# Vidvox/hap

Measured on AMD Instinct MI355X. Metric: RGBA GB/s + frames/sec, 8K Hap Q encode+decode, higher is better.
Workload: dtype u8; 1 GPU; C4: 7680x4320 0x1, 24 chunks, Snappy, 60-frame stream, device-resident; fragment_index=True, parallelism=single GPU

## Files before the change

hap_amd/csrc/bc_encode_core.hpp:

```cpp
#pragma once
#include <hip/hip_runtime.h>
#include <stdint.h>

namespace hapbc {

constexpr int kFmtDXT1 = 0, kFmtDXT5 = 1, kFmtYCoCg = 2, kFmtRGTC1 = 3;
constexpr int kFmtYCoCgAlpha = 4;

__device__ __forceinline__ int mad24(int a, int b, int c)
{
    int r;
    asm("v_mad_i32_i24 %0, %1, %2, %3" : "=v"(r) : "v"(a), "v"(b), "v"(c));
    return r;
}
template <int K>
__device__ __forceinline__ int mad24k(int a, int c)
{
    int r;
    asm("v_mad_i32_i24 %0, %1, %2, %3" : "=v"(r) : "v"(a), "i"(K), "v"(c));
    return r;
}

__device__ __forceinline__ int quant5(int v) { int t = mad24k<31>(v, 128); return (t + (t >> 8)) >> 8; }
__device__ __forceinline__ int quant6(int v) { int t = mad24k<63>(v, 128); return (t + (t >> 8)) >> 8; }
__device__ __forceinline__ int expand5(int q) { return (q << 3) | (q >> 2); }
__device__ __forceinline__ int expand6(int q) { return (q << 2) | (q >> 4); }


__device__ __forceinline__ unsigned ramp_codes(unsigned w)
{
    return w ^ (~((w >> 1) | (w >> 2)) & 0x249249u);
}

__device__ __forceinline__ uint2 alpha_block(const int (&a)[16])
{
    int lo = a[0], hi = a[0];
#pragma unroll
    for (int i = 1; i < 16; i++) {
        lo = min(lo, a[i]);
        hi = max(hi, a[i]);
    }
    const int a0 = hi, a1 = lo;
    unsigned lo24 = 0, hi24 = 0;
    if (a0 != a1) {
        const int d = a0 - a1;
        unsigned q = (unsigned)(524288.0f * __builtin_amdgcn_rcpf((float)d));
        const int rem = 524288 - (int)__umul24(q, (unsigned)d);
        q += (rem >= d ? 1u : 0u) - (rem < 0 ? 1u : 0u);
        const unsigned m = q + 1u;
        const int neg_m14 = -(int)(14u * m);
        const int start = mad24(a0, (int)(14u * m), (int)__umul24((unsigned)max(d - 6, 0), m)) + (1 << 20);
#pragma unroll
        for (int i = 0; i < 16; i++) {
            const unsigned r1 = (unsigned)mad24(a[i], neg_m14, start) >> 20;
            if (i < 8)
                lo24 = __builtin_amdgcn_alignbit(r1, lo24, 3);
            else
                hi24 = __builtin_amdgcn_alignbit(r1, hi24, 3);
        }
        lo24 = ramp_codes(lo24 >> 8);
        hi24 = ramp_codes(hi24 >> 8);
    }
    const unsigned long long bits = (unsigned long long)lo24 | ((unsigned long long)hi24 << 24);
    const unsigned long long v = (unsigned long long)(unsigned)a0 | ((unsigned long long)(unsigned)a1 << 8) | (bits << 16);
    return make_uint2((unsigned)v, (unsigned)(v >> 32));
}

struct projection {
    unsigned adir;
    unsigned flip;
    int start;
    int top;
    unsigned m24;
};

__device__ __forceinline__ unsigned index_scale(unsigned len2)
{
    unsigned m = (unsigned)(50331648.0f * __builtin_amdgcn_rcpf((float)len2));
    const int rem = (int)(50331648u - m * len2);
    m += (rem >= (int)len2 ? 1u : 0u) - (rem < 0 ? 1u : 0u);
    return m;
}

template <int CHANNELS = 3>
__device__ __forceinline__ projection make_projection(unsigned p0, unsigned p1)
{
    projection pr;
    int dir[CHANNELS];
    unsigned adir = 0, flip = 0;
    int neg = 0, base = 0;
#pragma unroll
    for (int c = 0; c < CHANNELS; c++) {
        const int a = (int)((p0 >> (8 * c)) & 255u), b = (int)((p1 >> (8 * c)) & 255u);
        dir[c] = a - b;
        const int ad = abs(dir[c]);
        adir |= (unsigned)ad << (8 * c);
        flip |= (dir[c] < 0 ? 0xFFu : 0u) << (8 * c);
        neg += dir[c] < 0 ? ad : 0;
        base = mad24(b, dir[c], base);
    }
    const unsigned len2 = __builtin_amdgcn_udot4(adir, adir, 0u, false);
    const unsigned sixth = __umulhi(len2, 0xAAAAAAABu) >> 2;
    pr.adir = adir;
    pr.flip = flip;
    pr.start = (int)sixth - base - 255 * neg;
    pr.top = (int)(len2 + sixth);
    pr.m24 = index_scale(len2);
    return pr;
}

template <bool FLIPPED = false>
__device__ __forceinline__ unsigned project4(const unsigned (&px)[16], const projection &pr)
{
    unsigned pos2 = 0;
#pragma unroll
    for (int i = 0; i < 16; i++) {
        const unsigned q = FLIPPED ? px[i] : px[i] ^ pr.flip;
        const int t = (int)__builtin_amdgcn_udot4(q, pr.adir, (unsigned)pr.start, false);
        const int pos = min(max(__mul24(t, (int)pr.m24) >> 24, 0), 3);
        pos2 = __builtin_amdgcn_alignbit((unsigned)pos, pos2, 2);
    }
    const unsigned hi = pos2 & 0xAAAAAAAAu;
    const unsigned idx = (hi ^ ((pos2 << 1) & 0xAAAAAAAAu)) | ((~hi >> 1) & 0x55555555u);
    return idx;
}

__device__ __forceinline__ unsigned pack3(int a, int b, int c) { return (unsigned)a | ((unsigned)b << 8) | ((unsigned)c << 16); }

__device__ __forceinline__ unsigned expand_565(unsigned c, bool blue)
{
    return pack3(expand5(c >> 11), expand6((c >> 5) & 63), blue ? expand5(c & 31) : 0);
}

__device__ __forceinline__ uint2 colour_block(const unsigned (&px)[16])
{
    int lo[3] = {255, 255, 255}, hi[3] = {0, 0, 0};
#pragma unroll
    for (int i = 0; i < 16; i++) {
#pragma unroll
        for (int c = 0; c < 3; c++) {
            const int v = (int)((px[i] >> (8 * c)) & 255u);
            lo[c] = min(lo[c], v);
            hi[c] = max(hi[c], v);
        }
    }
    int cov_rg = 0, cov_bg = 0;
    const int mr = lo[0] + hi[0], mg = lo[1] + hi[1], mb = lo[2] + hi[2];
#pragma unroll
    for (int i = 0; i < 16; i++) {
        const int dr = 2 * (int)(px[i] & 255u) - mr;
        const int dg = 2 * (int)((px[i] >> 8) & 255u) - mg;
        const int db = 2 * (int)((px[i] >> 16) & 255u) - mb;
        cov_rg = mad24(dr, dg, cov_rg);
        cov_bg = mad24(db, dg, cov_bg);
    }
#pragma unroll
    for (int c = 0; c < 3; c++) {
        const int inset = (hi[c] - lo[c]) >> 4;
        lo[c] += inset;
        hi[c] -= inset;
    }
    const int ar = cov_rg < 0 ? lo[0] : hi[0], br = cov_rg < 0 ? hi[0] : lo[0];
    const int ab = cov_bg < 0 ? lo[2] : hi[2], bb = cov_bg < 0 ? hi[2] : lo[2];
    const unsigned qa = (unsigned)(quant5(ar) << 11 | quant6(hi[1]) << 5 | quant5(ab));
    const unsigned qb = (unsigned)(quant5(br) << 11 | quant6(lo[1]) << 5 | quant5(bb));
    const unsigned c0 = max(qa, qb), c1 = min(qa, qb);
    unsigned idx = 0;
    if (c0 != c1)
        idx = project4(px, make_projection(expand_565(c0, true), expand_565(c1, true)));
    return make_uint2(c0 | (c1 << 16), idx);
}

typedef unsigned short pk_u16 __attribute__((ext_vector_type(2)));
typedef short pk_i16 __attribute__((ext_vector_type(2)));

__device__ __forceinline__ uint2 ycocg_colour_block(const unsigned (&cc)[16])
{
    pk_u16 lo = __builtin_bit_cast(pk_u16, cc[0]), hi = lo;
#pragma unroll
    for (int i = 1; i < 16; i++) {
        const pk_u16 v = __builtin_bit_cast(pk_u16, cc[i]);
        lo = __builtin_elementwise_min(lo, v);
        hi = __builtin_elementwise_max(hi, v);
    }
    int lo_o = lo.x, hi_o = hi.x, lo_g = lo.y, hi_g = hi.y;
    const int m = max(max(128 - lo_o, hi_o - 128), max(128 - lo_g, hi_g - 128));
    const int s = m <= 31 ? 4 : (m <= 63 ? 2 : 1);
    int prod = 0;
    pk_u16 sums = {0, 0};
#pragma unroll
    for (int i = 0; i < 16; i++) {
        int r;
        asm("v_mad_i32_i16 %0, %1, %1, %2 op_sel:[0,1,0,0]" : "=v"(r) : "v"(cc[i]), "v"(prod));
        prod = r;
        sums += __builtin_bit_cast(pk_u16, cc[i]);
    }
    const int mo = lo_o + hi_o, mg = lo_g + hi_g;
    const int cov = 4 * prod - 2 * mg * (int)sums.x - 2 * mo * (int)sums.y + 16 * mo * mg;
    lo_o = (lo_o - 128) * s + 128; hi_o = (hi_o - 128) * s + 128;
    lo_g = (lo_g - 128) * s + 128; hi_g = (hi_g - 128) * s + 128;
    int ins = (hi_o - lo_o) >> 4; lo_o += ins; hi_o -= ins;
    ins = (hi_g - lo_g) >> 4; lo_g += ins; hi_g -= ins;
    const int ag = cov < 0 ? lo_g : hi_g, bg = cov < 0 ? hi_g : lo_g;
    const int qo_a = quant5(hi_o), qo_b = quant5(lo_o), qg_a = quant6(ag), qg_b = quant6(bg);
    const unsigned qa = (unsigned)(qo_a << 11 | qg_a << 5 | (s - 1));
    const unsigned qb = (unsigned)(qo_b << 11 | qg_b << 5 | (s - 1));
    const unsigned c0 = max(qa, qb), c1 = min(qa, qb);
    unsigned idx = 0;
    if (c0 != c1) {
        const bool sw = qa < qb;
        const int eo_a = expand5(qo_a), eo_b = expand5(qo_b), eg_a = expand6(qg_a), eg_b = expand6(qg_b);
        const int d_o = sw ? eo_b - eo_a : eo_a - eo_b, d_g = sw ? eg_b - eg_a : eg_a - eg_b;
        const int p1_o = sw ? eo_a : eo_b, p1_g = sw ? eg_a : eg_b;
        const unsigned len2 = (unsigned)mad24(d_o, d_o, __mul24(d_g, d_g));
        const int sixth = (int)(__umulhi(len2, 0xAAAAAAABu) >> 2);
        const unsigned m24 = index_scale(len2);
        const int centre = 128 - 128 * s;
        const int K = mad24(d_o, centre - p1_o, mad24(d_g, centre - p1_g, sixth));
        const pk_i16 dir2 = {(short)d_o, (short)d_g};
        constexpr int kDotOffset = 1 << 17;
        const unsigned sm = (unsigned)s * m24;
        const unsigned Km = (unsigned)(K - s * kDotOffset) * m24;
        unsigned pos2 = 0;
#pragma unroll
        for (int i = 0; i < 16; i++) {
            unsigned dot;
            asm("v_dot2_i32_i16 %0, %1, %2, %3\n\ts_nop 2" : "=v"(dot) : "v"(cc[i]), "v"(__builtin_bit_cast(unsigned, dir2)), "s"(kDotOffset));
            const int pos = min(max((int)(__umul24(dot, sm) + Km) >> 24, 0), 3);
            pos2 = __builtin_amdgcn_alignbit((unsigned)pos, pos2, 2);
        }
        const unsigned hi = pos2 & 0xAAAAAAAAu;
        idx = (hi ^ ((pos2 << 1) & 0xAAAAAAAAu)) | ((~hi >> 1) & 0x55555555u);
    }
    return make_uint2(c0 | (c1 << 16), idx);
}

template <int FMT>
__device__ __forceinline__ uint4 block_of(const unsigned (&p)[16])
{
    if (FMT == kFmtRGTC1) {
        int a[16];
#pragma unroll
        for (int i = 0; i < 16; i++)
            a[i] = (int)(p[i] >> 24);
        const uint2 ab = alpha_block(a);
        return make_uint4(ab.x, ab.y, 0u, 0u);
    } else if (FMT == kFmtDXT1) {
        unsigned px[16];
#pragma unroll
        for (int i = 0; i < 16; i++)
            px[i] = p[i] & 0x00FFFFFFu;
        const uint2 cb = colour_block(px);
        return make_uint4(cb.x, cb.y, 0u, 0u);
    } else if (FMT == kFmtDXT5) {
        int a[16];
        unsigned px[16];
#pragma unroll
        for (int i = 0; i < 16; i++) {
            a[i] = (int)(p[i] >> 24);
            px[i] = p[i] & 0x00FFFFFFu;
        }
        const uint2 ab = alpha_block(a), cb = colour_block(px);
        return make_uint4(ab.x, ab.y, cb.x, cb.y);
    } else {
        int y[16];
        unsigned cc[16];
#pragma unroll
        for (int i = 0; i < 16; i++) {
            const unsigned q = p[i];
            y[i] = (int)(__builtin_amdgcn_udot4(q, 0x00010201u, 2u, false) >> 2);
            const unsigned co2 = __builtin_amdgcn_udot4(q ^ 0x00FF0000u, 0x00010001u, 2u, false);
            const unsigned cg4 = __builtin_amdgcn_udot4(q ^ 0x00FF00FFu, 0x00010201u, 4u, false);
            const pk_u16 raw = __builtin_bit_cast(pk_u16, co2 | (cg4 << 16)), sh = {1, 2};
            cc[i] = __builtin_bit_cast(unsigned, (pk_u16)(raw >> sh));
        }
        const uint2 ab = alpha_block(y), cb = ycocg_colour_block(cc);
        return make_uint4(ab.x, ab.y, cb.x, cb.y);
    }
}

}
```

Measured before the change: 2557 GB/s.

## Recenter YCoCg chroma to signed values and batch clamped dot-product index projection

```diff
diff --git a/hap_amd/csrc/bc_encode_core.hpp b/hap_amd/csrc/bc_encode_core.hpp
--- a/hap_amd/csrc/bc_encode_core.hpp
+++ b/hap_amd/csrc/bc_encode_core.hpp
@@ -32,6 +32,7 @@
     return w ^ (~((w >> 1) | (w >> 2)) & 0x249249u);
 }
 
+template <int BIAS = 0>
 __device__ __forceinline__ uint2 alpha_block(const int (&a)[16])
 {
     int lo = a[0], hi = a[0];
@@ -62,7 +63,7 @@
         hi24 = ramp_codes(hi24 >> 8);
     }
     const unsigned long long bits = (unsigned long long)lo24 | ((unsigned long long)hi24 << 24);
-    const unsigned long long v = (unsigned long long)(unsigned)a0 | ((unsigned long long)(unsigned)a1 << 8) | (bits << 16);
+    const unsigned long long v = (unsigned long long)(unsigned)(a0 + (a1 << 8) + BIAS * 257) | (bits << 16);
     return make_uint2((unsigned)v, (unsigned)(v >> 32));
 }
 
@@ -109,20 +110,45 @@
     return pr;
 }
 
+#define HAPBC_CLAMPED_DOTS(OP)                                                                                           \
+    asm(OP " %0, %4, %8, %9\n\t" OP " %1, %5, %8, %9\n\t" OP " %2, %6, %8, %9\n\t" OP " %3, %7, %8, %9\n\t"              \
+        "v_med3_i32 %0, %0, 0, %10\n\tv_med3_i32 %1, %1, 0, %10\n\tv_med3_i32 %2, %2, 0, %10\n\tv_med3_i32 %3, %3, 0, %10" \
+        : "=&v"(t[0]), "=&v"(t[1]), "=&v"(t[2]), "=&v"(t[3])                                                             \
+        : "v"(q0), "v"(q1), "v"(q2), "v"(q3), "v"(dir), "v"(start), "v"(top))
+__device__ __forceinline__ void clamped_dot4(unsigned (&t)[4], unsigned q0, unsigned q1, unsigned q2, unsigned q3, unsigned dir, int start, int top)
+{
+    HAPBC_CLAMPED_DOTS("v_dot4_u32_u8");
+}
+__device__ __forceinline__ void clamped_dot2(unsigned (&t)[4], unsigned q0, unsigned q1, unsigned q2, unsigned q3, unsigned dir, int start, int top)
+{
+    HAPBC_CLAMPED_DOTS("v_dot2_i32_i16");
+}
+#undef HAPBC_CLAMPED_DOTS
+
+template <typename DOTS>
+__device__ __forceinline__ unsigned gather_indices(unsigned m24, DOTS dots)
+{
+    const unsigned m30 = m24 << 6;
+    unsigned pos2 = 0;
+#pragma unroll
+    for (int g = 3; g >= 0; g--) {
+        unsigned t[4];
+        dots(t, 4 * g);
+#pragma unroll
+        for (int k = 3; k >= 0; k--)
+            pos2 = __builtin_amdgcn_alignbit(pos2, t[k] * m30, 30);
+    }
+    const unsigned hi = pos2 & 0xAAAAAAAAu;
+    return (hi ^ ((pos2 << 1) & 0xAAAAAAAAu)) | ((~hi >> 1) & 0x55555555u);
+}
+
 template <bool FLIPPED = false>
 __device__ __forceinline__ unsigned project4(const unsigned (&px)[16], const projection &pr)
 {
-    unsigned pos2 = 0;
-#pragma unroll
-    for (int i = 0; i < 16; i++) {
-        const unsigned q = FLIPPED ? px[i] : px[i] ^ pr.flip;
-        const int t = (int)__builtin_amdgcn_udot4(q, pr.adir, (unsigned)pr.start, false);
-        const int pos = min(max(__mul24(t, (int)pr.m24) >> 24, 0), 3);
-        pos2 = __builtin_amdgcn_alignbit((unsigned)pos, pos2, 2);
-    }
-    const unsigned hi = pos2 & 0xAAAAAAAAu;
-    const unsigned idx = (hi ^ ((pos2 << 1) & 0xAAAAAAAAu)) | ((~hi >> 1) & 0x55555555u);
-    return idx;
+    return gather_indices(pr.m24, [&](unsigned (&t)[4], int i) {
+        clamped_dot4(t, FLIPPED ? px[i] : px[i] ^ pr.flip, FLIPPED ? px[i + 1] : px[i + 1] ^ pr.flip,
+                     FLIPPED ? px[i + 2] : px[i + 2] ^ pr.flip, FLIPPED ? px[i + 3] : px[i + 3] ^ pr.flip, pr.adir, pr.start, pr.top);
+    });
 }
 
 __device__ __forceinline__ unsigned pack3(int a, int b, int c) { return (unsigned)a | ((unsigned)b << 8) | ((unsigned)c << 16); }
@@ -176,29 +202,29 @@
 
 __device__ __forceinline__ uint2 ycocg_colour_block(const unsigned (&cc)[16])
 {
-    pk_u16 lo = __builtin_bit_cast(pk_u16, cc[0]), hi = lo;
+    pk_i16 lo = __builtin_bit_cast(pk_i16, cc[0]), hi = lo;
 #pragma unroll
     for (int i = 1; i < 16; i++) {
-        const pk_u16 v = __builtin_bit_cast(pk_u16, cc[i]);
+        const pk_i16 v = __builtin_bit_cast(pk_i16, cc[i]);
         lo = __builtin_elementwise_min(lo, v);
         hi = __builtin_elementwise_max(hi, v);
     }
     int lo_o = lo.x, hi_o = hi.x, lo_g = lo.y, hi_g = hi.y;
-    const int m = max(max(128 - lo_o, hi_o - 128), max(128 - lo_g, hi_g - 128));
+    const int m = max(max(-lo_o, hi_o), max(-lo_g, hi_g));
     const int s = m <= 31 ? 4 : (m <= 63 ? 2 : 1);
     int prod = 0;
-    pk_u16 sums = {0, 0};
+    pk_i16 sums = {0, 0};
 #pragma unroll
     for (int i = 0; i < 16; i++) {
         int r;
         asm("v_mad_i32_i16 %0, %1, %1, %2 op_sel:[0,1,0,0]" : "=v"(r) : "v"(cc[i]), "v"(prod));
         prod = r;
-        sums += __builtin_bit_cast(pk_u16, cc[i]);
+        sums += __builtin_bit_cast(pk_i16, cc[i]);
     }
     const int mo = lo_o + hi_o, mg = lo_g + hi_g;
     const int cov = 4 * prod - 2 * mg * (int)sums.x - 2 * mo * (int)sums.y + 16 * mo * mg;
-    lo_o = (lo_o - 128) * s + 128; hi_o = (hi_o - 128) * s + 128;
-    lo_g = (lo_g - 128) * s + 128; hi_g = (hi_g - 128) * s + 128;
+    lo_o = lo_o * s + 128; hi_o = hi_o * s + 128;
+    lo_g = lo_g * s + 128; hi_g = hi_g * s + 128;
     int ins = (hi_o - lo_o) >> 4; lo_o += ins; hi_o -= ins;
     ins = (hi_g - lo_g) >> 4; lo_g += ins; hi_g -= ins;
     const int ag = cov < 0 ? lo_g : hi_g, bg = cov < 0 ? hi_g : lo_g;
@@ -215,24 +241,24 @@
         const unsigned len2 = (unsigned)mad24(d_o, d_o, __mul24(d_g, d_g));
         const int sixth = (int)(__umulhi(len2, 0xAAAAAAABu) >> 2);
         const unsigned m24 = index_scale(len2);
-        const int centre = 128 - 128 * s;
-        const int K = mad24(d_o, centre - p1_o, mad24(d_g, centre - p1_g, sixth));
-        const pk_i16 dir2 = {(short)d_o, (short)d_g};
-        constexpr int kDotOffset = 1 << 17;
-        const unsigned sm = (unsigned)s * m24;
-        const unsigned Km = (unsigned)(K - s * kDotOffset) * m24;
-        unsigned pos2 = 0;
-#pragma unroll
-        for (int i = 0; i < 16; i++) {
-            unsigned dot;
-            asm("v_dot2_i32_i16 %0, %1, %2, %3\n\ts_nop 2" : "=v"(dot) : "v"(cc[i]), "v"(__builtin_bit_cast(unsigned, dir2)), "s"(kDotOffset));
-            const int pos = min(max((int)(__umul24(dot, sm) + Km) >> 24, 0), 3);
-            pos2 = __builtin_amdgcn_alignbit((unsigned)pos, pos2, 2);
-        }
-        const unsigned hi = pos2 & 0xAAAAAAAAu;
-        idx = (hi ^ ((pos2 << 1) & 0xAAAAAAAAu)) | ((~hi >> 1) & 0x55555555u);
+        const int K = mad24(d_o, 128 - p1_o, mad24(d_g, 128 - p1_g, sixth));
+        const unsigned dir2 = ((unsigned)(d_o * s) & 0xFFFFu) | ((unsigned)(d_g * s) << 16);
+        const int top = (int)len2 + sixth;
+        idx = gather_indices(m24, [&](unsigned (&t)[4], int i) { clamped_dot2(t, cc[i], cc[i + 1], cc[i + 2], cc[i + 3], dir2, K, top); });
     }
     return make_uint2(c0 | (c1 << 16), idx);
+}
+
+__device__ __forceinline__ void chroma4(unsigned (&raw)[4], int q0, int q1, int q2, int q3)
+{
+    unsigned co[4];
+    asm("v_dot4_i32_i8 %4, %8, %12, 1\n\tv_dot4_i32_i8 %0, %8, %13, 2\n\t"
+        "v_dot4_i32_i8 %5, %9, %12, 1\n\tv_dot4_i32_i8 %1, %9, %13, 2\n\t"
+        "v_dot4_i32_i8 %6, %10, %12, 1\n\tv_dot4_i32_i8 %2, %10, %13, 2\n\t"
+        "v_dot4_i32_i8 %7, %11, %12, 1\n\tv_dot4_i32_i8 %3, %11, %13, 2\n\t"
+        "v_perm_b32 %0, %0, %4, %14\n\tv_perm_b32 %1, %1, %5, %14\n\tv_perm_b32 %2, %2, %6, %14\n\tv_perm_b32 %3, %3, %7, %14"
+        : "=&v"(raw[0]), "=&v"(raw[1]), "=&v"(raw[2]), "=&v"(raw[3]), "=&v"(co[0]), "=&v"(co[1]), "=&v"(co[2]), "=&v"(co[3])
+        : "v"(q0), "v"(q1), "v"(q2), "v"(q3), "s"(0x00FF0001), "s"(0x00FF02FF), "s"(0x05040100));
 }
 
 template <int FMT>
@@ -267,14 +293,19 @@
         unsigned cc[16];
 #pragma unroll
         for (int i = 0; i < 16; i++) {
-            const unsigned q = p[i];
-            y[i] = (int)(__builtin_amdgcn_udot4(q, 0x00010201u, 2u, false) >> 2);
-            const unsigned co2 = __builtin_amdgcn_udot4(q ^ 0x00FF0000u, 0x00010001u, 2u, false);
-            const unsigned cg4 = __builtin_amdgcn_udot4(q ^ 0x00FF00FFu, 0x00010201u, 4u, false);
-            const pk_u16 raw = __builtin_bit_cast(pk_u16, co2 | (cg4 << 16)), sh = {1, 2};
-            cc[i] = __builtin_bit_cast(unsigned, (pk_u16)(raw >> sh));
-        }
-        const uint2 ab = alpha_block(y), cb = ycocg_colour_block(cc);
+            y[i] = (int)__builtin_amdgcn_udot4(p[i], 0x00010201u, (unsigned)(2 - 512), false) >> 2;
+        }
+#pragma unroll
+        for (int i = 0; i < 16; i += 4) {
+            unsigned raw[4];
+            chroma4(raw, (int)(p[i] ^ 0x80808080u), (int)(p[i + 1] ^ 0x80808080u), (int)(p[i + 2] ^ 0x80808080u), (int)(p[i + 3] ^ 0x80808080u));
+#pragma unroll
+            for (int k = 0; k < 4; k++) {
+                const pk_i16 sh = {1, 2};
+                cc[i + k] = __builtin_bit_cast(unsigned, (pk_i16)(__builtin_bit_cast(pk_i16, raw[k]) >> sh));
+            }
+        }
+        const uint2 ab = alpha_block<128>(y), cb = ycocg_colour_block(cc);
         return make_uint4(ab.x, ab.y, cb.x, cb.y);
     }
 }
```

Measured after the change: 2602 GB/s, median of 6. +1.8%, better.
